# byu-magicc/VI-EKF

Measured on AMD Instinct MI355X. Metric: EKF steps/sec (IMU-rate propagate + N_feat updates), batch=1024, N_feat=50, higher is better.
Workload: dtype f64

## Files before the change

vi_ekf_amd/csrc/viekf_resident_common.hpp:

```cpp
#pragma once
#include <type_traits>

#include "viekf_instance_rows.hpp"
#include "viekf_kernels_stream.hpp"

namespace viekf {

constexpr int RES_FMT_LOAD_PACKED = 1, RES_FMT_STORE_PACKED = 2, RES_FMT_P_ONLY = 4;

#ifndef RES_INLINE
#define RES_INLINE __forceinline__
#endif
constexpr int ZK = 9;
constexpr int ZS = 26;

__host__ __device__ inline int res_mcap(int N) { return N > 64 ? 80 : 64; }

constexpr int RES_SM_SQRTQU = 64, RES_SM_QXB = 70;

struct ResLds {
  int xs, Kt, Wt, Praw, lam, sm, fixadd, fixset, Z, phiff, Abb, Gb, Phibb, Mbb, Gdb, Pbb, T16, xdb, ctx, Pbc, PhibbT, Pd, PsiP, Pi, Xi, AvG, Lbc, mslot, mseq, mz, mR, img_len, total;
  __host__ __device__ ResLds(int N, int n, int nxs, bool staged) {
    const int nf = 3 * N;
    int o = 0;
    auto take = [&](int cnt) { int r = o; o += (cnt + 1) & ~1; return r; };
    xs = take(nxs);
    lam = take(n);
    sm = take(staged ? 64 + 22 : 64);
    fixadd = take(2 * (N > 0 ? N : 1)); fixset = take(2 * (N > 0 ? N : 1));
    Z = take(nf * ZS > 4 * n ? nf * ZS : 4 * n);
    phiff = take(9 * (N > 0 ? N : 1));
    const int u0 = o;
    Abb = take(256); Gb = take(96); Phibb = take(256); PhibbT = take(256); Gdb = take(96); T16 = take(256);
    PsiP = take(ZK * 16); Pi = take(ZK * ZK); Xi = take(ZK * 16); AvG = take(18);
    const int uprop = o;
    o = u0;
    Kt = take(2 * n); Wt = take(2 * n);
    Praw = take(4 * n > 256 ? 4 * n : 256);
    Pd = take(4 * (N > 0 ? N : 1));
    if (uprop > o) o = uprop;
    img_len = o - Z;
    Mbb = take(256); Pbb = take(256);
    xdb = take(16);
    ctx = take((int)((sizeof(BodyCtx) + 7) / 8));
    Pbc = take(nf * 16);
    Lbc = take(48);
    const int mc = res_mcap(N);
    mslot = take(mc / 2); mseq = take(mc); mz = take(2 * mc); mR = take(4 * mc);
    total = o;
  }
};
__device__ __forceinline__ void wave_lds_sync() {
  __builtin_amdgcn_fence(__ATOMIC_RELEASE, "wavefront");
  __builtin_amdgcn_wave_barrier();
  __builtin_amdgcn_fence(__ATOMIC_ACQUIRE, "wavefront");
}
__device__ __forceinline__ int opaque(int v) { asm volatile("" : "+v"(v)); return v; }
typedef double v2f64 __attribute__((ext_vector_type(2)));
__device__ __forceinline__ double2 lds_ld2(const double* p) {
  const v2f64 v = *reinterpret_cast<const v2f64*>(p);
  return make_double2(v.x, v.y);
}
template <bool ON>
__device__ __forceinline__ void group_fence() {
  if (ON) {
    asm volatile("" ::: "memory");
    __builtin_amdgcn_sched_barrier(0);
  }
}
__device__ __forceinline__ double uniform_f64(double v) {
  const unsigned long long u = __double_as_longlong(v);
  const unsigned lo = __builtin_amdgcn_readfirstlane((unsigned)u), hi = __builtin_amdgcn_readfirstlane((unsigned)(u >> 32));
  return __longlong_as_double(((unsigned long long)hi << 32) | lo);
}

#ifdef VIEKF_STAMPS
#define RES_STAMP(S_, who, idx)                                                                  \
  do {                                                                                           \
    if ((S_).b == 0 && (who)) {                                                                  \
      __builtin_amdgcn_sched_barrier(0);                                                         \
      reinterpret_cast<unsigned long long*>((S_).stamps)[(idx)] = __builtin_amdgcn_s_memtime();  \
      __builtin_amdgcn_sched_barrier(0);                                                         \
    }                                                                                            \
  } while (0)
#else
#define RES_STAMP(S_, who, idx) do {} while (0)
#endif

#ifdef VIEKF_ISA_MARKS
#define RES_MARK(name)                          \
  do {                                          \
    __builtin_amdgcn_sched_barrier(0);          \
    asm volatile("; @@MARK " name);             \
    __builtin_amdgcn_sched_barrier(0);          \
  } while (0)
#else
#define RES_MARK(name) do {} while (0)
#endif

#ifdef VIEKF_ABLATE
#define RES_ABLATE(S_, bit) (((S_).dbg & (bit)) != 0)
#else
#define RES_ABLATE(S_, bit) false
#endif

typedef __attribute__((address_space(3))) volatile int lds_vint_t;

struct ResShared {
  double *xs, *Kt, *Wt, *Praw, *lam, *sm, *fixadd, *fixset, *Z, *phiff, *Abb, *Gb, *Phibb, *Mbb, *Gdb, *Pbb, *T16,
      *xdb, *Pbc, *PhibbT, *Pd, *PsiP, *Pi, *Xi, *AvG, *Lbc, *mz, *mR;
  int* mslot;
  int2* mseq;
  BodyCtx* ctx;
  int N, n, nf, len, M, mstride, do_prop, b, dbg, kp, B, img_len, mcap;
  int fmt;
  long si, so;
  double* stamps;
};

template <int RB, int TW>
__device__ __forceinline__ void res_words(const int* __restrict__ resmap, int t, int (&w)[RB]) {
#pragma unroll
  for (int ia = 0; ia < RB; ia++) w[ia] = resmap[ia * TW + t];
}
constexpr bool res_batched_loads(int RB, int NW) { return NW != 7 && RB != 8; }
__device__ __forceinline__ bool res_word_blk(int e, int& I, int& J) {
  I = e & 0xff;
  J = (e >> 8) & 0xff;
  return (e >> 16) != 0;
}

__device__ __forceinline__ int res_next_valid(const ResShared& S, int from) {
  int m = from;
  while (m < S.M && S.mslot[m] < 0) m++;
  return m;
}

}
```

vi_ekf_amd/csrc/viekf_resident_prop.hpp:

```cpp
#pragma once
#include "viekf_resident_common.hpp"

namespace viekf {


__device__ RES_INLINE void res_body_phase(const double* xs, const double* u, const DevParams* p, BodyCtx* ctx,
                                            double* xdb, double* Abb, double* Gb) {
  double ub[6];
  q_rota(p->q_b_u, u, ub);
  q_rota(p->q_b_u, u + 3, ub + 3);
  BodyCtx c;
  body_ctx(xs, ub, *p, c);
  body_dynamics<false>(c, *p, xdb, Abb, Gb);
  *ctx = c;
}

__device__ RES_INLINE void res_feature_phase(int f, int len, double dt, double* xs, const BodyCtx* ctx, double* Z,
                                             double* phiff) {
  double* z0 = Z + (3 * f) * ZS;
  if (f < len) {
    double xd3[3], Afv[9], Afg[9], Aff[9];
    const double qz[4] = {xs[xZ + 5 * f], xs[xZ + 5 * f + 1], xs[xZ + 5 * f + 2], xs[xZ + 5 * f + 3]};
    const double rho = xs[xZ + 5 * f + 4];
    const BodyCtx c = *ctx;
    feature_dynamics(qz, rho, c, xd3, Afv, Afg, Aff);
    double Aff2[9];
    mm<3, 3, 3>(Aff, Aff, Aff2);
#pragma unroll
    for (int e = 0; e < 9; e++) {
      const double id = (e == 0 || e == 4 || e == 8) ? 1.0 : 0.0;
      phiff[9 * f + e] = id + Aff[e] * dt + Aff2[e] * (0.5 * dt * dt);
    }
#pragma unroll
    for (int r = 0; r < 3; r++)
#pragma unroll
      for (int c3 = 0; c3 < 3; c3++) {
        z0[r * ZS + 2 * c3] = Afv[r * 3 + c3]; z0[r * ZS + 2 * (3 + c3)] = Afg[r * 3 + c3]; z0[r * ZS + 2 * (6 + c3)] = Aff[r * 3 + c3];
      }
    double qn[4];
    q_feat_boxplus_fast(qz, xd3[0] * dt, xd3[1] * dt, qn);
    double* xf = xs + xZ + 5 * f;
    xf[0] = qn[0]; xf[1] = qn[1]; xf[2] = qn[2]; xf[3] = qn[3];
    xf[4] = rho + xd3[2] * dt;
  } else {
    for (int r = 0; r < 3; r++)
      for (int e = 0; e < 9; e++) z0[r * ZS + 2 * e] = 0.0;
    for (int e = 0; e < 9; e++) phiff[9 * f + e] = (e == 0 || e == 4 || e == 8) ? 1.0 : 0.0;
  }
}

__device__ RES_INLINE void res_feature_expand_row(int f, int r, double dt, double* Z, const double* Gb, const double* AvG,
                                                  const double* sqrtQu) {
  const double* z0 = Z + (3 * f) * ZS;
  double* zr = Z + (3 * f + r) * ZS;
  auto raw = [&](int row, int c) { return z0[row * ZS + 2 * c]; };
  const double a0 = raw(r, 6), a1 = raw(r, 7), a2 = raw(r, 8);
  double AAv[3], AAg[3], A2r[3], afv[3], afg[3];
#pragma unroll
  for (int j = 0; j < 3; j++) {
    afv[j] = raw(r, j); afg[j] = raw(r, 3 + j);
    AAv[j] = a0 * raw(0, j) + a1 * raw(1, j) + a2 * raw(2, j);
    AAg[j] = a0 * raw(0, 3 + j) + a1 * raw(1, 3 + j) + a2 * raw(2, 3 + j);
    A2r[j] = a0 * raw(0, 6 + j) + a1 * raw(1, 6 + j) + a2 * raw(2, 6 + j);
  }
  const double ar[3] = {a0, a1, a2};
  double mff[3];
#pragma unroll
  for (int j = 0; j < 3; j++) mff[j] = ((j == r) ? 1.0 : 0.0) + ar[j] * (0.5 * dt) + A2r[j] * (dt * dt * (1.0 / 6.0));
#pragma unroll
  for (int k = 0; k < 6; k++) {
    double a = 0.0, b = 0.0;
#pragma unroll
    for (int j = 0; j < 3; j++) {
      a += (afv[j] + (dt * (1.0 / 3.0)) * AAv[j]) * Gb[(dxVEL + j) * 6 + k];
      b += afv[j] * AvG[j * 6 + k];
    }
    double g = a * (0.5 * dt) + b * (dt * dt * (1.0 / 6.0));
    if (k >= 3) g += mff[0] * raw(0, k) + mff[1] * raw(1, k) + mff[2] * raw(2, k);
    zr[18 + k] = g * dt * sqrtQu[k];
  }
#pragma unroll
  for (int j = 0; j < 3; j++) {
    zr[2 * j + 1] = (afv[j] + (0.5 * dt) * AAv[j]) * dt;
    zr[2 * (3 + j) + 1] = afv[j] * (0.5 * dt * dt);
    zr[2 * (6 + j) + 1] = (afg[j] + (0.5 * dt) * AAg[j]) * dt;
  }
}

__device__ RES_INLINE void res_fix_depth(double* xf, const DevParams* p, double* fixadd_slot, double* fixset_slot,
                                         double* fixany, unsigned* flag) {
  double rho = xf[4];
  fix_depth_rule(rho, 1.0 / (2.0 * p->min_depth), *flag, [&](double e2) { *fixadd_slot = e2; *fixany = 1.0; },
                 [&] { *fixset_slot = 1.0; *fixany = 1.0; });
  xf[4] = rho;
}


template <int TW, bool LDSC = false>
__device__ __forceinline__ void res_prop_setup(const StreamArgs& a, const ResShared& S, int tid) {
  const int nf = S.nf, N = S.N;
  const DevParams& prm = *a.dp;
  double* Pbc = S.Pbc; double* Pbb = S.Pbb;
  double* Z = S.Z; double* phiff = S.phiff;
  double* Phibb = S.Phibb; double* Mbb = S.Mbb; double* Gdb = S.Gdb; double* T16 = S.T16;
  __syncthreads();
  const double dt = S.sm[42];

  for (int e = tid; e < nf; e += TW) res_feature_expand_row(e / 3, e % 3, dt, Z, S.Gb, S.AvG, LDSC ? S.sm + RES_SM_SQRTQU : prm.sqrtQu);
  for (int e = TW - 1 - tid; e < 256; e += TW) {
    const int r = e >> 4, c = e & 15;
    double a2 = 0.0;
#pragma unroll 4
    for (int k = 0; k < 16; k++) a2 += S.Abb[r * 16 + k] * S.Abb[k * 16 + c];
    const double id = (r == c) ? 1.0 : 0.0, av = S.Abb[e];
    Mbb[e] = id + av * (0.5 * dt) + a2 * (dt * dt * (1.0 / 6.0));
    const double ph = id + av * dt + a2 * (0.5 * dt * dt);
    Phibb[e] = ph;
    S.PhibbT[c * 16 + r] = ph;
  }
  for (int e = TW - 1 - tid; e < ZK * 16; e += TW) {
    const int q = e >> 4, c = e & 15;
    double v;
    if (q < 3) v = Pbb[(dxVEL + q) * 16 + c];
    else if (q >= 6) v = Pbb[(dxB_G + q - 6) * 16 + c];
    else {
      v = 0.0;
#pragma unroll 4
      for (int k = 0; k < 16; k++) v += S.Abb[(dxVEL + q - 3) * 16 + k] * Pbb[k * 16 + c];
    }
    S.PsiP[e] = v;
  }
  for (int e = tid; e < 16 * N; e += TW) {
    const int f = e >> 4, k = e & 15;
    const double* ff = phiff + 9 * f;
    double* pc = Pbc + (3 * f) * 16 + k;
    const double p0 = pc[0], p1 = pc[16], p2 = pc[32];
    pc[0] = ff[0] * p0 + ff[1] * p1 + ff[2] * p2;
    pc[16] = ff[3] * p0 + ff[4] * p1 + ff[5] * p2;
    pc[32] = ff[6] * p0 + ff[7] * p1 + ff[8] * p2;
  }
  __syncthreads();

  for (int e = tid; e < 256; e += TW) {
    const int r = e >> 4, c = e & 15;
    double sv = 0.0;
#pragma unroll 4
    for (int k = 0; k < 16; k++) sv += Phibb[r * 16 + k] * Pbb[k * 16 + c];
    T16[e] = sv;
  }
  for (int e = TW - 1 - tid; e < 96; e += TW) {
    const int r = e / 6, k = e % 6;
    double sv = 0.0;
#pragma unroll 4
    for (int c = 0; c < 16; c++) sv += Mbb[r * 16 + c] * S.Gb[c * 6 + k];
    Gdb[e] = sv * dt * (LDSC ? S.sm[RES_SM_SQRTQU + k] : prm.sqrtQu[k]);
  }
  for (int e = tid; e < ZK * ZK; e += TW) {
    const int q = e / ZK, j = e - q * ZK;
    const double* pr = S.PsiP + q * 16;
    double v;
    if (j < 3) v = pr[dxVEL + j];
    else if (j >= 6) v = pr[dxB_G + j - 6];
    else {
      v = 0.0;
#pragma unroll 4
      for (int k = 0; k < 16; k++) v += pr[k] * S.Abb[(dxVEL + j - 3) * 16 + k];
    }
    S.Pi[e] = v;
  }
  __syncthreads();

  {
    const int lane = tid & 63, wv = tid >> 6, lr = lane & 15, lk = lane >> 4;
    double bv[7];
    int aoff[7];
#pragma unroll
    for (int sk = 0; sk < 7; sk++) {
      const int k = 4 * sk + lk, c = k - ZK;
      double v = 0.0;
      if (lr < ZK) {
        if (k < ZK) v = 0.5 * S.Pi[k * ZK + lr];
        else if (c < 16) v = (lr < 3) ? ((c == dxVEL + lr) ? 1.0 : 0.0)
                           : ((lr >= 6) ? ((c == dxB_G + lr - 6) ? 1.0 : 0.0) : S.Abb[(dxVEL + lr - 3) * 16 + c]);
      }
      bv[sk] = v;
      aoff[sk] = (k < ZK) ? (2 * k + 1) : ((c < 16) ? (0x100 | c) : -1);
    }
    for (int t = wv; t * 16 < nf; t += TW / 64) {
      const int ar = min(16 * t + lr, nf - 1);
      v4f64 acc = {0.0, 0.0, 0.0, 0.0};
#pragma unroll
      for (int sk = 0; sk < 7; sk++) {
        const int o = aoff[sk];
        const double av = (o < 0) ? 0.0 : ((o & 0x100) ? Pbc[ar * 16 + (o & 0xff)] : Z[ar * ZS + o]);
        acc = __builtin_amdgcn_mfma_f64_16x16x4f64(av, bv[sk], acc, 0, 0, 0);
      }
#pragma unroll
      for (int r4 = 0; r4 < 4; r4++) {
        const int row = 16 * t + lk + 4 * r4;
        if (row < nf && lr < ZK) Z[row * ZS + 2 * lr] = acc[r4];
      }
    }
  }
  for (int e = TW - 1 - tid; e < ZK * 16; e += TW) {
    const int q = e >> 4, c = e & 15;
    double v;
    if (q < 3) v = T16[c * 16 + dxVEL + q];
    else if (q >= 6) v = T16[c * 16 + dxB_G + q - 6];
    else {
      v = 0.0;
#pragma unroll 4
      for (int k = 0; k < 16; k++) v += S.Abb[(dxVEL + q - 3) * 16 + k] * T16[c * 16 + k];
    }
    S.Xi[e] = v;
  }
}

template <int TW, bool LDSC = false>
__device__ __forceinline__ void res_prop_body(const StreamArgs& a, const ResShared& S, int tid) {
  const int nf = S.nf;
  double* Pbc = S.Pbc;
  const double* Z = S.Z; double* Gdb = S.Gdb; double* T16 = S.T16;
  {
    const int lane = tid & 63, wv = tid >> 6, lr = lane & 15, lk = lane >> 4;
    constexpr int step = TW / 64;
    double bph[4], bdx[4];
    int zoff[4];
#pragma unroll
    for (int sk = 0; sk < 4; sk++) {
      const int k = 4 * sk + lk;
      bph[sk] = S.PhibbT[k * 16 + lr];
      bdx[sk] = (k < ZK) ? S.Xi[k * 16 + lr] : ((k < ZK + 6) ? Gdb[lr * 6 + (k - ZK)] : 0.0);
      zoff[sk] = (k < ZK) ? (2 * k + 1) : ((k < ZK + 6) ? (18 + k - ZK) : -1);
    }
    for (int t = wv; t * 16 < nf; t += 2 * step) {
      const int t1 = t + step;
      const int r0 = min(16 * t + lr, nf - 1), r1 = min(16 * t1 + lr, nf - 1);
      double a0[8], a1[8];
#pragma unroll
      for (int sk = 0; sk < 4; sk++) {
        a0[sk] = Pbc[r0 * 16 + 4 * sk + lk]; a1[sk] = Pbc[r1 * 16 + 4 * sk + lk];
        a0[4 + sk] = (zoff[sk] >= 0) ? Z[r0 * ZS + zoff[sk]] : 0.0;
        a1[4 + sk] = (zoff[sk] >= 0) ? Z[r1 * ZS + zoff[sk]] : 0.0;
      }
      v4f64 acc0 = {0.0, 0.0, 0.0, 0.0}, acc1 = {0.0, 0.0, 0.0, 0.0};
#pragma unroll
      for (int sk = 0; sk < 8; sk++) {
        const double bv = sk < 4 ? bph[sk] : bdx[sk - 4];
        acc0 = __builtin_amdgcn_mfma_f64_16x16x4f64(a0[sk], bv, acc0, 0, 0, 0);
        acc1 = __builtin_amdgcn_mfma_f64_16x16x4f64(a1[sk], bv, acc1, 0, 0, 0);
      }
#pragma unroll
      for (int r4 = 0; r4 < 4; r4++) {
        const int row0 = 16 * t + lk + 4 * r4, row1 = 16 * t1 + lk + 4 * r4;
        if (row0 < nf) Pbc[row0 * 16 + lr] = acc0[r4];
        if (row1 < nf) Pbc[row1 * 16 + lr] = acc1[r4];
      }
    }
  }
  if (tid < 64) {
    const int lr = tid & 15, lk = tid >> 4;
    v4f64 acc = {0.0, 0.0, 0.0, 0.0};
#pragma unroll
    for (int sk = 0; sk < 4; sk++) {
      const int k = 4 * sk + lk;
      acc = __builtin_amdgcn_mfma_f64_16x16x4f64(T16[lr * 16 + k], S.PhibbT[k * 16 + lr], acc, 0, 0, 0);
    }
#pragma unroll
    for (int sk = 0; sk < 2; sk++) {
      const int k = 4 * sk + lk;
      const double gv = (k < 6) ? Gdb[lr * 6 + k] : 0.0;
      acc = __builtin_amdgcn_mfma_f64_16x16x4f64(gv, gv, acc, 0, 0, 0);
    }
#pragma unroll
    for (int r4 = 0; r4 < 4; r4++) {
      const int r = lk + 4 * r4, c = lr;
      S.Mbb[r * 16 + c] = acc[r4] + ((r == c) ? (LDSC ? S.sm[RES_SM_QXB + r] : a.Qx[r]) : 0.0);
    }
  }
}

}
```

vi_ekf_amd/csrc/viekf_resident_worker.hpp:

```cpp
#pragma once
#include "viekf_resident_prop.hpp"

namespace viekf {


struct StoreChunk { int f0, f1, rb, h; };
__device__ __forceinline__ bool store_chunk_at(int f0, int N, int n, int img_len, StoreChunk& c) {
  if (f0 >= N) return false;
  c.f0 = f0;
  c.rb = (16 + 3 * f0) & ~1;
  c.h = ((n + 1) & ~1) - c.rb;
  c.f1 = min(N, f0 + max(1, img_len / (3 * c.h)));
  return true;
}
template <int T>
__device__ __forceinline__ void res_store_chunk(const StreamArgs& a, const ResShared& S, const StoreChunk& c, int tid) {
  const int n = S.n, ld = a.ld;
  double* P = a.P_out + S.so * n * ld;
  const double* img = S.Z;
  const int ncol = 3 * (c.f1 - c.f0), lane = tid & 63, w = tid >> 6;
  constexpr int NWV = T / 64;
  if ((n & 1) == 0) {
#pragma unroll 2
    for (int col = w; col < ncol; col += NWV) {
      const int j = 16 + 3 * c.f0 + col;
      const double* src = img + col * c.h - c.rb;
      for (int i0 = c.rb; i0 < n; i0 += 256) {
        double2 v[2];
#pragma unroll
        for (int u = 0; u < 2; u++) v[u] = lds_ld2(src + min(i0 + 2 * (lane + 64 * u), n - 2));
#pragma unroll
        for (int u = 0; u < 2; u++) {
          const int i = i0 + 2 * (lane + 64 * u);
          if (i < n && i + 1 >= j) *reinterpret_cast<double2*>(P + i + (long)j * ld) = v[u];
        }
      }
    }
  } else {
#pragma unroll 2
    for (int col = w; col < ncol; col += NWV) {
      const int j = 16 + 3 * c.f0 + col;
      const double* src = img + col * c.h - c.rb;
      for (int i = c.rb + lane; i < n; i += 64)
        if (i >= j) P[i + (long)j * ld] = src[i];
    }
  }
}

template <int RB, int TW>
__device__ __forceinline__ void res_store_packed(double* img, const double (&pb)[RB][9], const double* Pbc, const double* Pbb,
                                                 int N, int t) {
  constexpr ResPack K(0, RB, TW / 64);
  v2f64* dst = reinterpret_cast<v2f64*>(img) + t;
#pragma unroll
  for (int p = 0; p < K.npair; p++) {
    v2f64 v;
    v.x = pb[(2 * p) / 9][(2 * p) % 9];
    v.y = pb[(2 * p + 1) / 9][(2 * p + 1) % 9];
    dst[p * TW] = v;
  }
  if ((9 * RB) & 1) img[K.single + t] = pb[RB - 1][8];
  v2f64* gc = reinterpret_cast<v2f64*>(img + K.pbc);
  for (int e = t; e < 24 * N; e += TW) gc[e] = *reinterpret_cast<const v2f64*>(Pbc + 2 * e);
  v2f64* gb = reinterpret_cast<v2f64*>(img + K.pbc + 48 * N);
  for (int e = t; e < 128; e += TW) gb[e] = *reinterpret_cast<const v2f64*>(Pbb + 2 * e);
}
__device__ __forceinline__ void res_body_items(const ResShared& S, const double* kP, bool run, int id, int nthreads,
                                               int first, int last, int slot2, double* rawdst) {
  const double* wP = kP + 2 * S.n;
  double* Pbc = S.Pbc;
  const int j2 = ((first + id) & 7) * 2;
  double2 cw0 = {}, cw1 = {}, cl[3] = {};
  if (run) {
    cw0 = lds_ld2(wP + 2 * j2);
    cw1 = lds_ld2(wP + 2 * j2 + 2);
#pragma unroll
    for (int q = 0; q < 3; q++) cl[q] = lds_ld2(S.Lbc + 16 * q + j2);
  }
#pragma unroll 1
  for (int item = first + id; item < last; item += nthreads) {
    const int g = item >> 3;
    double2 cpv[3];
#pragma unroll
    for (int q = 0; q < 3; q++) cpv[q] = lds_ld2(Pbc + (3 * g + q) * 16 + j2);
    if (run) {
      double2 cki[3];
#pragma unroll
      for (int q = 0; q < 3; q++) cki[q] = lds_ld2(kP + 2 * (16 + 3 * g + q));
#pragma unroll
      for (int q = 0; q < 3; q++) {
        cpv[q].x = fma(-cl[q].x, fma(cki[q].y, cw0.y, cki[q].x * cw0.x), cpv[q].x);
        cpv[q].y = fma(-cl[q].y, fma(cki[q].y, cw1.y, cki[q].x * cw1.x), cpv[q].y);
        *reinterpret_cast<double2*>(Pbc + (3 * g + q) * 16 + j2) = cpv[q];
      }
    }
    if (g == slot2) {
      double* st = rawdst + 2 * j2;
      *reinterpret_cast<double2*>(st) = make_double2(cpv[0].x, cpv[1].x);
      *reinterpret_cast<double2*>(st + 2) = make_double2(cpv[0].y, cpv[1].y);
    }
  }
}
template <int RB, int TW, bool MP, int T = TW + 64, bool ZU = false, bool BL = true>
__device__ __forceinline__ void res_worker(const StreamArgs& a, const ResShared& S, int tid) {
  const int N = S.N, n = S.n, ld = a.ld, nf = S.nf, len = S.len;
  double* P = a.P + S.si * n * ld;
  const int tid_ = tid;
  constexpr int NWV = TW / 64;
  const DevParams& prm = *a.dp;
  double* Pbc = S.Pbc;
  double* Pbb = S.Pbb;
  const int* __restrict__ resmap = a.resmap;
  auto blk = [&](const int (&w)[RB], int t, int ia, int& I, int& J) -> bool {
    return res_word_blk(BL ? w[ia] : resmap[ia * TW + t], I, J);
  };
  const bool own_diag = tid_ < N;

  double pb[RB][9];
  const bool ldp = (S.fmt & RES_FMT_LOAD_PACKED) != 0;
  if (ldp) {
    const int t = opaque(tid_);
    constexpr ResPack K(0, RB, TW / 64);
    const v2f64* gc = reinterpret_cast<const v2f64*>(P + K.pbc);
    for (int e = t; e < 24 * N; e += TW) *reinterpret_cast<v2f64*>(Pbc + 2 * e) = gc[e];
    const v2f64* gb = reinterpret_cast<const v2f64*>(P + K.pbc + 48 * N);
    for (int e = t; e < 128; e += TW) *reinterpret_cast<v2f64*>(Pbb + 2 * e) = gb[e];
  }
  {
    const int tq = opaque(tid_);
    int ew[RB];
    if (BL) res_words<RB, TW>(resmap, tq, ew);
#pragma unroll
    for (int ia = 0; ia < RB; ia++) {
      int I, J;
      blk(ew, tq, ia, I, J);
      const bool up = I < J;
      const int br = 16 + 3 * (up ? J : I), bc = 16 + 3 * (up ? I : J);
      const unsigned cbase = (unsigned)(br + bc * ld);
      const unsigned base = ldp ? 2u * (unsigned)tq : cbase, base1 = ldp ? (unsigned)tq : cbase;
#pragma unroll
      for (int s = 0; s < 3; s++)
#pragma unroll
        for (int r = 0; r < 3; r++) {
          const int rr = (I == J) ? max(r, s) : (up ? s : r), cc = (I == J) ? min(r, s) : (up ? r : s);
          constexpr ResPack K(0, RB, TW / 64);
          const int q = ia * 9 + r * 3 + s;
          const unsigned offp = (unsigned)K.elem(q, 0), offc = (unsigned)(rr + cc * ld);
          pb[ia][r * 3 + s] = P[((q < 2 * K.npair) ? base : base1) + (ldp ? offp : offc)];
        }
    }
    for (int e = tid; !ldp && e < nf * 16; e += TW) {
      const int k = e / nf, row = e - k * nf;
      Pbc[row * 16 + k] = P[(16 + row) + (long)k * ld];
    }
    for (int e = tid; !ldp && e < 256; e += TW) {
      const int r = e & 15, c = e >> 4;
      Pbb[r * 16 + c] = P[max(r, c) + (long)min(r, c) * ld];
    }
  }

  auto sym_diag = [&]() {
    if (own_diag) { pb[0][3] = pb[0][1]; pb[0][6] = pb[0][2]; pb[0][7] = pb[0][5]; }
  };
  sym_diag();
  double Lff[9];
  {
    const double lf[3] = {a.lambda[16], a.lambda[17], a.lambda[18]};
#pragma unroll
    for (int r = 0; r < 3; r++)
#pragma unroll
      for (int s = 0; s < 3; s++) Lff[r * 3 + s] = uniform_f64(prm.use_partial_update ? (lf[s] + lf[r] - lf[r] * lf[s]) : 1.0);
  }
  const bool partial = prm.use_partial_update != 0;
  int par = 0;
  constexpr int NSV = (T - TW) / 64;
  auto fix_word = [&](int mb) -> double { return (NSV > 1) ? S.sm[40 + mb] + S.sm[36 + mb] : S.sm[40 + mb]; };
  RES_STAMP(S, tid == 0, 64);
  __syncthreads();
  RES_STAMP(S, tid == 0, 65);

  const int nkp = MP ? S.kp : 1;
  int eu[RB];
  if (S.do_prop)
   for (int kp = 0; kp < nkp; kp++) {
    const int tk = MP ? opaque(tid) : tid;
    const double* Z = S.Z; double* phiff = S.phiff;
    int ep[RB];
    double qd[3];
    if (BL) {
      const int tq = opaque(tid_);
      res_words<RB, TW>(resmap, tq, ep);
#pragma unroll
      for (int r = 0; r < 3; r++) qd[r] = a.Qx[16 + 3 * min(tq, N - 1) + r];
    }
    if (MP || !BL) res_prop_setup<TW>(a, S, tk);
    else res_prop_setup<TW, true>(a, S, tk);
    RES_STAMP(S, tid == 0, 66);
    __syncthreads();
    RES_STAMP(S, tid == 0, 67);

#pragma unroll
    for (int ia = 0; ia < RB; ia++) {
      const int tq = BL ? 0 : opaque(tid_);
      int I, J;
      const bool v = blk(ep, tq, ia, I, J);
      const double* fj = phiff + 9 * J;
#pragma unroll
      for (int r = 0; r < 3; r++) {
        const double p0 = pb[ia][r * 3 + 0], p1 = pb[ia][r * 3 + 1], p2 = pb[ia][r * 3 + 2];
#pragma unroll
        for (int s = 0; s < 3; s++) pb[ia][r * 3 + s] = p0 * fj[s * 3 + 0] + p1 * fj[s * 3 + 1] + p2 * fj[s * 3 + 2];
      }
      const double* fi = phiff + 9 * I;
#pragma unroll
      for (int s = 0; s < 3; s++) {
        const double p0 = pb[ia][0 * 3 + s], p1 = pb[ia][1 * 3 + s], p2 = pb[ia][2 * 3 + s];
#pragma unroll
        for (int r = 0; r < 3; r++) pb[ia][r * 3 + s] = fi[r * 3 + 0] * p0 + fi[r * 3 + 1] * p1 + fi[r * 3 + 2] * p2;
      }
      if (BL) {
        if (ia == 0 && own_diag) { pb[0][0] += qd[0]; pb[0][4] += qd[1]; pb[0][8] += qd[2]; }
      } else if (v && I == J) {
        pb[ia][0] += a.Qx[16 + 3 * I + 0];
        pb[ia][4] += a.Qx[16 + 3 * I + 1];
        pb[ia][8] += a.Qx[16 + 3 * I + 2];
      }
      __builtin_amdgcn_sched_barrier(0);
      if (RB > 4) {
#pragma unroll
        for (int e = 0; e < 9; e++) asm volatile("" : "+v"(pb[ia][e]));
      }
      group_fence<(RB > 4)>();
    }
    RES_STAMP(S, tid == 0, 68);
    int zoff[RB];
    {
      const int tq = BL ? 0 : opaque(tid_);
#pragma unroll
      for (int ia = 0; ia < RB; ia++) {
        int I, J;
        blk(ep, tq, ia, I, J);
        zoff[ia] = (3 * I * ZS) | ((3 * J * ZS) << 16);
      }
    }
    auto contract = [&](int k, auto crossed) {
      constexpr bool CROSS = decltype(crossed)::value;
#pragma unroll
      for (int ia = 0; ia < RB; ia++) {
        const double* zi = Z + (zoff[ia] & 0xffff) + 2 * k;
        const double* zj = Z + (zoff[ia] >> 16) + 2 * k;
        double2 xv[3], yv[3];
#pragma unroll
        for (int r = 0; r < 3; r++) xv[r] = lds_ld2(zi + r * ZS);
#pragma unroll
        for (int s = 0; s < 3; s++) yv[s] = lds_ld2(zj + s * ZS);
#pragma unroll
        for (int r = 0; r < 3; r++)
#pragma unroll
          for (int s = 0; s < 3; s++) {
            double acc = pb[ia][r * 3 + s];
            acc = fma(xv[r].x, CROSS ? yv[s].y : yv[s].x, acc);
            acc = fma(xv[r].y, CROSS ? yv[s].x : yv[s].y, acc);
            pb[ia][r * 3 + s] = acc;
          }
        if (ia & 1) group_fence<(RB > 4)>();
      }
    };
#pragma unroll 1
    for (int k = 0; k < ZK; k++) contract(k, std::true_type{});
#pragma unroll 1
    for (int k = ZK; k < ZK + 3; k++) contract(k, std::false_type{});
    sym_diag();
    RES_STAMP(S, tid == 0, 69);
    if (BL && !MP) res_words<RB, TW>(resmap, opaque(tid_), eu);
    if (MP) res_prop_body<TW, BL>(a, S, tk);
    par ^= 1;
    RES_STAMP(S, tid == 0, 70);
    __syncthreads();
    for (int e = tk; e < 256; e += TW) { const int r = e >> 4, c = e & 15; Pbb[e] = S.Mbb[min(r, c) * 16 + max(r, c)]; }
    if (MP && kp + 1 < nkp && own_diag && tid_ < len && fix_word(par ^ 1) != 0.0) {
      const int mb = par ^ 1, I = tid_;
      const double ad = S.fixadd[mb * N + I], st = S.fixset[mb * N + I];
      if (ad != 0.0) { pb[0][8] += ad; S.fixadd[mb * N + I] = 0.0; }
      if (st != 0.0) { pb[0][8] = prm.P0_feat[2]; S.fixset[mb * N + I] = 0.0; }
    }
   }

  int Ib[RB], Jb[RB];
  bool vb[RB];
  if (BL && (MP || !S.do_prop)) res_words<RB, TW>(resmap, opaque(tid_), eu);
#pragma unroll
  for (int ia = 0; ia < RB; ia++) vb[ia] = blk(eu, tid_, ia, Ib[ia], Jb[ia]);
  const double p0rr = uniform_f64(prm.P0_feat[2]);
  auto bb_mask = [&](int r, int c) -> double { const double lr_ = S.lam[r], lc_ = S.lam[c]; return partial ? (lc_ + lr_ - lr_ * lc_) : 1.0; };
  double bbL0 = 1.0, bbL1 = 1.0;
  {
    constexpr int BBT0 = (TW >= 128) ? 128 : TW;
    const int ib0 = tid - (TW - BBT0);
    if (ib0 >= 0 && ib0 < 128) { bbL0 = bb_mask(ib0 >> 3, (ib0 & 7) * 2); bbL1 = bb_mask(ib0 >> 3, (ib0 & 7) * 2 + 1); }
  }
  auto apply_fixes = [&](int mb, double pending) {
    if (pending == 0.0) return;
    if (own_diag && tid_ < len) {
      VIEKF_COLD_BEGIN();
      const int I = tid_;
      const double ad = S.fixadd[mb * N + I], st = S.fixset[mb * N + I];
      if (ad != 0.0) { pb[0][8] += ad; S.fixadd[mb * N + I] = 0.0; }
      if (st != 0.0) { pb[0][8] = p0rr; S.fixset[mb * N + I] = 0.0; }
      VIEKF_COLD_END();
    }
  };
  auto extract_cols = [&](int slot, double* Pw) {
#pragma unroll
    for (int ia = 0; ia < RB; ia++) {
      const int I = Ib[ia], J = Jb[ia];
      const bool asrow = J == slot;
      const bool ascol = !asrow && I == slot;
      if (vb[ia] && (asrow || ascol)) {
        const int base = 16 + 3 * (asrow ? I : J);
        const double a0 = pb[ia][0], a1 = asrow ? pb[ia][1] : pb[ia][3];
        const double b0 = asrow ? pb[ia][3] : pb[ia][1], b1 = pb[ia][4];
        const double c0 = asrow ? pb[ia][6] : pb[ia][2], c1 = asrow ? pb[ia][7] : pb[ia][5];
        *reinterpret_cast<double2*>(Pw + 2 * (base + 0)) = make_double2(a0, a1);
        *reinterpret_cast<double2*>(Pw + 2 * (base + 1)) = make_double2(b0, b1);
        *reinterpret_cast<double2*>(Pw + 2 * (base + 2)) = make_double2(c0, c1);
      }
    }
  };

  int m = res_next_valid(S, 0);
  if (own_diag) {
    *reinterpret_cast<double2*>(S.Pd + 4 * tid_) = make_double2(pb[0][0], pb[0][1]);
    *reinterpret_cast<double2*>(S.Pd + 4 * tid_ + 2) = make_double2(pb[0][3], pb[0][4]);
  }
  int2 sq = S.mseq[min(m, S.mcap - 1)];
  if (m < S.M) {
    apply_fixes(par ^ 1, fix_word(par ^ 1));
    const int s0 = S.mslot[m];
    extract_cols(s0, S.Praw);
    if (sq.y >= 0) extract_cols(sq.y, S.Praw + 2 * n);
    const int e = opaque(tid);
    if (e < 16) {
      const int sf = (e < 8) ? s0 : sq.y, ijj = (e & 7) * 2;
      if (sf >= 0) {
        const double2 q0 = lds_ld2(Pbc + (3 * sf) * 16 + ijj);
        const double2 q1 = lds_ld2(Pbc + (3 * sf + 1) * 16 + ijj);
        double* d = S.Praw + ((e < 8) ? 0 : 2 * n) + 2 * ijj;
        *reinterpret_cast<double2*>(d) = make_double2(q0.x, q1.x);
        *reinterpret_cast<double2*>(d + 2) = make_double2(q0.y, q1.y);
      }
    }
  }
  RES_STAMP(S, tid == 0, 71);
  __syncthreads();
  __syncthreads();
  int it_ = 0;
  int cnt = 0;
  while (m < S.M) {
    const int mnext = sq.x;
    RES_MARK("worker.phase_top");
    const double* kP = (cnt & 1) ? S.Z : S.Kt;
    const double* wP = kP + 2 * n;
    __builtin_amdgcn_s_setprio(1);
    const double fixpending = fix_word(par ^ 1);
    const double gflag = S.sm[50 + (cnt & 1)];
    const double nanw = (NSV > 1) ? S.sm[44 + cnt % 3] + S.sm[52 + cnt % 3] : S.sm[44 + cnt % 3];
    sq = S.mseq[min(mnext, S.mcap - 1)];
    RES_STAMP(S, tid == 0 && it_ < 8, 80 + 4 * it_ + 1);
    RES_STAMP(S, (tid & 63) == 0 && it_ == 3, 192 + 4 * (tid >> 6) + 0);
    const int it = tid;
    constexpr int GB = (RB <= 4) ? RB : 2;
    RES_MARK("worker.block_sweep");
    const bool gated = gflag != 0.0;
    const bool run = !gated && nanw == 0.0 && !RES_ABLATE(S, 1);
    bool fixed = false;
#pragma unroll
    for (int g0 = 0; g0 < RB; g0 += GB) {
      double2 kI[GB][3], wJ[GB][3];
#pragma unroll
      for (int ig = 0; ig < GB; ig++) {
        const int ia = (g0 + ig < RB) ? g0 + ig : RB - 1;
#pragma unroll
        for (int r = 0; r < 3; r++) kI[ig][r] = lds_ld2(kP + 2 * (16 + 3 * Ib[ia] + r));
#pragma unroll
        for (int s = 0; s < 3; s++) wJ[ig][s] = lds_ld2(wP + 2 * (16 + 3 * Jb[ia] + s));
      }
      if (!fixed) { apply_fixes(par ^ 1, fixpending); fixed = true; }
      if (run) {
#pragma unroll
        for (int ig = 0; ig < GB; ig++) {
          if (g0 + ig >= RB) continue;
          const int ia = g0 + ig;
#pragma unroll
          for (int r = 0; r < 3; r++)
#pragma unroll
            for (int s = 0; s < 3; s++) {
              if (ZU && !(r == 2 && s == 2)) {
                pb[ia][r * 3 + s] = fma(-kI[ig][r].y, wJ[ig][s].y, fma(-kI[ig][r].x, wJ[ig][s].x, pb[ia][r * 3 + s]));
              } else {
                const double t = fma(kI[ig][r].y, wJ[ig][s].y, kI[ig][r].x * wJ[ig][s].x);
                pb[ia][r * 3 + s] = fma(-Lff[r * 3 + s], t, pb[ia][r * 3 + s]);
              }
            }
        }
      }
      group_fence<(RB > GB)>();
    }
    sym_diag();
    RES_MARK("worker.column_extraction");
    RES_STAMP(S, tid == 0 && it_ < 8, 160 + 4 * it_ + 0);
    double* rawdst = S.Praw + (cnt & 1) * 2 * n;
    if (sq.y >= 0 && !RES_ABLATE(S, 4) && !(RES_ABLATE(S, 8) && (cnt & 1))) extract_cols(sq.y, rawdst);
    __builtin_amdgcn_s_setprio(0);
    RES_STAMP(S, tid == 0 && it_ < 8, 160 + 4 * it_ + 1);
    RES_STAMP(S, (tid & 63) == 0 && it_ == 3, 192 + 4 * (tid >> 6) + 2);
    __builtin_amdgcn_sched_barrier(0);
    RES_MARK("worker.body_items");
    res_body_items(S, kP, run, (it >= 64) ? it - 64 : it + TW - 64, TW, 0, 8 * N, sq.y, rawdst);
    RES_MARK("worker.body_block");
    if (run) {
      constexpr int BBT = (TW >= 128) ? 128 : TW;
#pragma unroll
      for (int ib = it - (TW - BBT); ib >= 0 && ib < 128; ib += BBT) {
        const int br = ib >> 3, bc2 = (ib & 7) * 2;
        double2 bpv = *reinterpret_cast<double2*>(Pbb + br * 16 + bc2);
        const double2 kr = lds_ld2(kP + 2 * br), wr = lds_ld2(wP + 2 * br);
        const double2 k0 = lds_ld2(kP + 2 * bc2), w0 = lds_ld2(wP + 2 * bc2);
        const double2 k1 = lds_ld2(kP + 2 * bc2 + 2), w1 = lds_ld2(wP + 2 * bc2 + 2);
        const double L0 = (BBT == 128) ? bbL0 : bb_mask(br, bc2), L1 = (BBT == 128) ? bbL1 : bb_mask(br, bc2 + 1);
        const bool up0 = br <= bc2, up1 = br <= bc2 + 1;
        const double2 ka = up0 ? kr : k0, wa = up0 ? w0 : wr;
        const double2 kb = up1 ? kr : k1, wb = up1 ? w1 : wr;
        bpv.x = fma(-L0, fma(ka.y, wa.y, ka.x * wa.x), bpv.x);
        bpv.y = fma(-L1, fma(kb.y, wb.y, kb.x * wb.x), bpv.y);
        *reinterpret_cast<double2*>(Pbb + br * 16 + bc2) = bpv;
      }
    }
    RES_MARK("worker.phase_tail");
    par ^= 1;
    cnt++;
    RES_STAMP(S, tid == 0 && it_ < 8, 80 + 4 * it_ + 2);
    RES_STAMP(S, (tid & 63) == 0 && it_ == 3, 192 + 4 * (tid >> 6) + 1);
    __syncthreads();
    RES_STAMP(S, tid == 0 && it_ < 8, 80 + 4 * it_ + 3);
    RES_STAMP(S, (tid & 63) == 0 && it_ == 3, 192 + 4 * (tid >> 6) + 3);
    it_++;
    m = mnext;
  }
  RES_MARK("worker.loop_end");
  apply_fixes(par ^ 1, fix_word(par ^ 1));
  RES_STAMP(S, tid == 0, 72);
  __syncthreads();

  P = a.P_out + S.so * n * ld;
  if (S.fmt & RES_FMT_STORE_PACKED) {
    res_store_packed<RB, TW>(P, pb, Pbc, Pbb, N, opaque(tid_));
  } else {
    int es[RB];
    if (BL) res_words<RB, TW>(resmap, opaque(tid_), es);
    for (int e = opaque(tid); e < nf * 16; e += TW) {
      const int k = e / nf, row = e - k * nf;
      P[(16 + row) + (long)k * ld] = Pbc[row * 16 + k];
    }
    for (int e = opaque(tid); e < 256; e += TW) P[(e >> 4) + (long)(e & 15) * ld] = Pbb[e];
    double* img = S.Z;
    const int gtid = threadIdx.x;
    RES_STAMP(S, tid == 0, 224);
    StoreChunk sc;
    int ch = 0;
    for (int f0 = 0; store_chunk_at(f0, N, n, S.img_len, sc); f0 = sc.f1, ch++) {
      const int f1 = sc.f1;
      const int tq = BL ? 0 : opaque(tid_);
#pragma unroll
      for (int ia = 0; ia < RB; ia++) {
        int I, J;
        if (blk(es, tq, ia, I, J)) {
          if (I >= J && J >= f0 && J < f1) {
            double* d = img + (3 * (J - f0)) * sc.h + (16 + 3 * I - sc.rb);
#pragma unroll
            for (int s = 0; s < 3; s++)
#pragma unroll
              for (int r = 0; r < 3; r++) d[s * sc.h + r] = pb[ia][r * 3 + s];
          }
          if (I < J && I >= f0 && I < f1) {
            double* d = img + (3 * (I - f0)) * sc.h + (16 + 3 * J - sc.rb);
#pragma unroll
            for (int r = 0; r < 3; r++)
#pragma unroll
              for (int s = 0; s < 3; s++) d[r * sc.h + s] = pb[ia][r * 3 + s];
          }
        }
      }
      RES_STAMP(S, tid == 0 && ch < 3, 225 + 4 * ch);
      __syncthreads();
      RES_STAMP(S, tid == 0 && ch < 3, 226 + 4 * ch);
      res_store_chunk<T>(a, S, sc, gtid);
      RES_STAMP(S, tid == 0 && ch < 3, 227 + 4 * ch);
      __syncthreads();
      RES_STAMP(S, tid == 0 && ch < 3, 228 + 4 * ch);
    }
  }
  RES_STAMP(S, tid == 0, 73);
}


}
```

Measured before the change: 3.281 million.

## Split P-block register loads into chunks issued during propagation setup phases

For selected (RB, waves) configurations without multi-prop, the worker loads only the first quarter of its per-thread covariance blocks up front. The remaining three quarters are issued through a hook at each barrier-separated phase of res_prop_setup, so global load latency overlaps the setup compute. The resmap words and Qx diagonal are hoisted and reused, and the Pbc/Pbb LDS staging is moved earlier. In exchange, more registers stay live across setup, and the path is gated to a handful of template configs.

```diff
diff --git a/vi_ekf_amd/csrc/viekf_resident_common.hpp b/vi_ekf_amd/csrc/viekf_resident_common.hpp
--- a/vi_ekf_amd/csrc/viekf_resident_common.hpp
+++ b/vi_ekf_amd/csrc/viekf_resident_common.hpp
@@ -124,6 +124,9 @@
   for (int ia = 0; ia < RB; ia++) w[ia] = resmap[ia * TW + t];
 }
 constexpr bool res_batched_loads(int RB, int NW) { return NW != 7 && RB != 8; }
+constexpr bool res_setup_under_load(int RB, int NW, bool MP) {
+  return res_batched_loads(RB, NW) && !MP && ((NW == 3 && (RB == 4 || RB == 6 || RB == 7)) || (NW == 6 && RB == 5));
+}
 __device__ __forceinline__ bool res_word_blk(int e, int& I, int& J) {
   I = e & 0xff;
   J = (e >> 8) & 0xff;
diff --git a/vi_ekf_amd/csrc/viekf_resident_prop.hpp b/vi_ekf_amd/csrc/viekf_resident_prop.hpp
--- a/vi_ekf_amd/csrc/viekf_resident_prop.hpp
+++ b/vi_ekf_amd/csrc/viekf_resident_prop.hpp
@@ -96,8 +96,9 @@
 }
 
 
-template <int TW, bool LDSC = false>
-__device__ __forceinline__ void res_prop_setup(const StreamArgs& a, const ResShared& S, int tid) {
+struct ResNoHook { template <class K> __device__ __forceinline__ void operator()(K) const {} };
+template <int TW, bool LDSC = false, class Hook = ResNoHook>
+__device__ __forceinline__ void res_prop_setup(const StreamArgs& a, const ResShared& S, int tid, const Hook& hook = Hook()) {
   const int nf = S.nf, N = S.N;
   const DevParams& prm = *a.dp;
   double* Pbc = S.Pbc; double* Pbb = S.Pbb;
@@ -105,6 +106,7 @@
   double* Phibb = S.Phibb; double* Mbb = S.Mbb; double* Gdb = S.Gdb; double* T16 = S.T16;
   __syncthreads();
   const double dt = S.sm[42];
+  hook(std::integral_constant<int, 0>{});
 
   for (int e = tid; e < nf; e += TW) res_feature_expand_row(e / 3, e % 3, dt, Z, S.Gb, S.AvG, LDSC ? S.sm + RES_SM_SQRTQU : prm.sqrtQu);
   for (int e = TW - 1 - tid; e < 256; e += TW) {
@@ -140,6 +142,7 @@
     pc[32] = ff[6] * p0 + ff[7] * p1 + ff[8] * p2;
   }
   __syncthreads();
+  hook(std::integral_constant<int, 1>{});
 
   for (int e = tid; e < 256; e += TW) {
     const int r = e >> 4, c = e & 15;
@@ -169,6 +172,7 @@
     S.Pi[e] = v;
   }
   __syncthreads();
+  hook(std::integral_constant<int, 2>{});
 
   {
     const int lane = tid & 63, wv = tid >> 6, lr = lane & 15, lk = lane >> 4;
diff --git a/vi_ekf_amd/csrc/viekf_resident_worker.hpp b/vi_ekf_amd/csrc/viekf_resident_worker.hpp
--- a/vi_ekf_amd/csrc/viekf_resident_worker.hpp
+++ b/vi_ekf_amd/csrc/viekf_resident_worker.hpp
@@ -103,6 +103,7 @@
 }
 template <int RB, int TW, bool MP, int T = TW + 64, bool ZU = false, bool BL = true>
 __device__ __forceinline__ void res_worker(const StreamArgs& a, const ResShared& S, int tid) {
+  constexpr bool SU = res_setup_under_load(RB, TW / 64, MP);
   const int N = S.N, n = S.n, ld = a.ld, nf = S.nf, len = S.len;
   double* P = a.P + S.si * n * ld;
   const int tid_ = tid;
@@ -118,6 +119,16 @@
 
   double pb[RB][9];
   const bool ldp = (S.fmt & RES_FMT_LOAD_PACKED) != 0;
+  double Lff[9];
+  bool partial_su = false;
+  if (SU) {
+    const double lf[3] = {a.lambda[16], a.lambda[17], a.lambda[18]};
+#pragma unroll
+    for (int r = 0; r < 3; r++)
+#pragma unroll
+      for (int s = 0; s < 3; s++) Lff[r * 3 + s] = uniform_f64(prm.use_partial_update ? (lf[s] + lf[r] - lf[r] * lf[s]) : 1.0);
+    partial_su = prm.use_partial_update != 0;
+  }
   if (ldp) {
     const int t = opaque(tid_);
     constexpr ResPack K(0, RB, TW / 64);
@@ -126,12 +137,32 @@
     const v2f64* gb = reinterpret_cast<const v2f64*>(P + K.pbc + 48 * N);
     for (int e = t; e < 128; e += TW) *reinterpret_cast<v2f64*>(Pbb + 2 * e) = gb[e];
   }
+  if (SU) {
+    for (int e = tid; !ldp && e < nf * 16; e += TW) {
+      const int k = e / nf, row = e - k * nf;
+      Pbc[row * 16 + k] = P[(16 + row) + (long)k * ld];
+    }
+    for (int e = tid; !ldp && e < 256; e += TW) {
+      const int r = e & 15, c = e >> 4;
+      Pbb[r * 16 + c] = P[max(r, c) + (long)min(r, c) * ld];
+    }
+  }
+  int ws[SU ? RB : 1];
+  double qs[3];
   {
     const int tq = opaque(tid_);
     int ew[RB];
     if (BL) res_words<RB, TW>(resmap, tq, ew);
-#pragma unroll
-    for (int ia = 0; ia < RB; ia++) {
+    if (SU) {
+#pragma unroll
+      for (int ia = 0; ia < RB; ia++) ws[ia] = ew[ia];
+      if (S.do_prop) {
+#pragma unroll
+        for (int r = 0; r < 3; r++) qs[r] = a.Qx[16 + 3 * min(tq, N - 1) + r];
+      }
+    }
+#pragma unroll
+    for (int ia = 0; ia < (SU ? RB / 4 : RB); ia++) {
       int I, J;
       blk(ew, tq, ia, I, J);
       const bool up = I < J;
@@ -149,29 +180,52 @@
           pb[ia][r * 3 + s] = P[((q < 2 * K.npair) ? base : base1) + (ldp ? offp : offc)];
         }
     }
-    for (int e = tid; !ldp && e < nf * 16; e += TW) {
+    for (int e = tid; !SU && !ldp && e < nf * 16; e += TW) {
       const int k = e / nf, row = e - k * nf;
       Pbc[row * 16 + k] = P[(16 + row) + (long)k * ld];
     }
-    for (int e = tid; !ldp && e < 256; e += TW) {
+    for (int e = tid; !SU && !ldp && e < 256; e += TW) {
       const int r = e & 15, c = e >> 4;
       Pbb[r * 16 + c] = P[max(r, c) + (long)min(r, c) * ld];
     }
   }
+
+  auto issue_chunk = [&](auto kc) {
+    constexpr int k = decltype(kc)::value + 1, lo = RB * k / 4, hi = RB * (k + 1) / 4;
+    const int tq = opaque(tid_);
+#pragma unroll
+    for (int ia = lo; ia < hi; ia++) {
+      int I, J;
+      res_word_blk(ws[SU ? ia : 0], I, J);
+      const bool up = I < J;
+      const int br = 16 + 3 * (up ? J : I), bc = 16 + 3 * (up ? I : J);
+      const unsigned cbase = (unsigned)(br + bc * ld);
+      const unsigned base = ldp ? 2u * (unsigned)tq : cbase, base1 = ldp ? (unsigned)tq : cbase;
+#pragma unroll
+      for (int s = 0; s < 3; s++)
+#pragma unroll
+        for (int r = 0; r < 3; r++) {
+          const int rr = (I == J) ? max(r, s) : (up ? s : r), cc = (I == J) ? min(r, s) : (up ? r : s);
+          constexpr ResPack K(0, RB, TW / 64);
+          const int q = ia * 9 + r * 3 + s;
+          const unsigned offp = (unsigned)K.elem(q, 0), offc = (unsigned)(rr + cc * ld);
+          pb[ia][r * 3 + s] = P[((q < 2 * K.npair) ? base : base1) + (ldp ? offp : offc)];
+        }
+    }
+  };
 
   auto sym_diag = [&]() {
     if (own_diag) { pb[0][3] = pb[0][1]; pb[0][6] = pb[0][2]; pb[0][7] = pb[0][5]; }
   };
-  sym_diag();
-  double Lff[9];
-  {
+  if (!SU) {
+    sym_diag();
     const double lf[3] = {a.lambda[16], a.lambda[17], a.lambda[18]};
 #pragma unroll
     for (int r = 0; r < 3; r++)
 #pragma unroll
       for (int s = 0; s < 3; s++) Lff[r * 3 + s] = uniform_f64(prm.use_partial_update ? (lf[s] + lf[r] - lf[r] * lf[s]) : 1.0);
   }
-  const bool partial = prm.use_partial_update != 0;
+  const bool partial = SU ? partial_su : prm.use_partial_update != 0;
   int par = 0;
   constexpr int NSV = (T - TW) / 64;
   auto fix_word = [&](int mb) -> double { return (NSV > 1) ? S.sm[40 + mb] + S.sm[36 + mb] : S.sm[40 + mb]; };
@@ -187,17 +241,28 @@
     const double* Z = S.Z; double* phiff = S.phiff;
     int ep[RB];
     double qd[3];
-    if (BL) {
+    if (SU) {
+#pragma unroll
+      for (int ia = 0; ia < RB; ia++) ep[ia] = ws[SU ? ia : 0];
+#pragma unroll
+      for (int r = 0; r < 3; r++) qd[r] = qs[r];
+    } else if (BL) {
       const int tq = opaque(tid_);
       res_words<RB, TW>(resmap, tq, ep);
 #pragma unroll
       for (int r = 0; r < 3; r++) qd[r] = a.Qx[16 + 3 * min(tq, N - 1) + r];
     }
     if (MP || !BL) res_prop_setup<TW>(a, S, tk);
+    else if (SU) res_prop_setup<TW, true>(a, S, tk, issue_chunk);
     else res_prop_setup<TW, true>(a, S, tk);
     RES_STAMP(S, tid == 0, 66);
     __syncthreads();
     RES_STAMP(S, tid == 0, 67);
+#ifdef VIEKF_STAMPS
+    asm volatile("s_waitcnt vmcnt(0)" ::: "memory");
+#endif
+    RES_STAMP(S, tid == 0, 74);
+    if (SU) sym_diag();
 
 #pragma unroll
     for (int ia = 0; ia < RB; ia++) {
@@ -286,6 +351,12 @@
     }
    }
 
+  if (SU && !S.do_prop) {
+    issue_chunk(std::integral_constant<int, 0>{});
+    issue_chunk(std::integral_constant<int, 1>{});
+    issue_chunk(std::integral_constant<int, 2>{});
+    sym_diag();
+  }
   int Ib[RB], Jb[RB];
   bool vb[RB];
   if (BL && (MP || !S.do_prop)) res_words<RB, TW>(resmap, opaque(tid_), eu);
```

New measurement: 3.330 million (median of 6 runs). 1.01x the previous value.
